# janelia-cosem/fibsem-optflow

Hardware: AMD Instinct MI355X
Metric: slice-pairs/sec (6k×4k, 5 scales, 30 warps) at 1/2/4/8 GPUs; % HBM roofline (higher is better)
Workload: dtype f32; 1 GPU; C2: one 6144x4096 u8 slice pair per GPU per step, nscales 5, warps 30, iterations 300, epsilon 0.01 (reference defaults otherwise); pair=6144x4096, parallelism=pairs sharded over 1 GPU(s), no data-path collective, pairs_in_flight_per_gpu=3, step=one batch of 3 pair(s) solved concurrently per GPU (one ctx + stream each), checks_per_pair=206

## Files before the change

### fibsem-optflow_amd/csrc/tvl1_engine.hip

```cpp
#include <hip/hip_runtime.h>
#include <sched.h>
#include <atomic>
#include <chrono>

#include <cfloat>
#include <cmath>
#include <cstdarg>
#include <cstdio>
#include <cstdlib>
#include <cstring>
#include <string>
#include <vector>

#include "../../include/tvl1.h"
#include "tvl1_plan.hpp"
#include "tvl1_walk.hpp"
#include "tvl1_kernels.hpp"
#include "tvl1_batch.hpp"
#include "tvl1_align_plan.hpp"
#include "tvl1_align.hpp"
#include "tvl1_stack.hpp"
#include "tvl1_shift.hpp"
#include "tvl1_fbcheck.hpp"
#include "tvl1_compose.hpp"
// ... 54 lines not shown
  unsigned long long *gate = nullptr;
  int spec = 1;
  int spec_trace = 0;
  unsigned long long check_seq = 0;
  int poll = 1;
  hipEvent_t ev_order = nullptr;
  hipEvent_t ev_switch = nullptr;
  hipStream_t last_stream = nullptr;
  bool last_stream_valid = false;
  struct Retired {
    char *p;
    std::vector<hipEvent_t> done;
  };
  std::vector<Retired> retired;
  std::vector<hipStream_t> streams;
  int roll_seg = 0;
  long roll_px4_min = 5000000;
  int roll_slots[kRollMax + 1][2][5] = {};
  int fill = 100;
  int fill_shared = 60;
  long roll_long_min = 0;
  int warp_ring_slots = 0;
  size_t buf_limit = ((size_t)1 << 31) - 4096;
  int fuse = 1;
  int tb4 = 1;
  long fuse_min = 4000000;
  int witer_slots = 0;
  int mid = 1;
  double mid_min = 1.1;
  int mid_slots = 0;
  int wi_nc = 2;
  int stages = 1;
  int stage_slots[kRollMax + 1] = {};
  int stages_fill = 0;
  char *barena = nullptr;
  size_t barena_bytes = 0;
  int bW = 0, bH = 0, bL = 0, bn = 0;
  int bws[TVL1_MAX_LEVELS] = {}, bhs[TVL1_MAX_LEVELS] = {};
  float *bI0s[TVL1_MAX_LEVELS] = {}, *bI1s[TVL1_MAX_LEVELS] = {};
  size_t bips[TVL1_MAX_LEVELS] = {};
  float *bU[2][2] = {}, *bP[2][4] = {}, *bC[3] = {};
  size_t bps = 0;
  double *bpartials = nullptr;
  int batch_fuse = 1;
  int batch_group = 1;
  int batch_store_pred = 1;
  int batch_px1_w = kBatchPx1W;
  int kb1_slots[kRollMax + 1] = {};
  int batch_seg_min = 128;
  int probe_lds = 0;
  int probe_wi_lds = 0;
  char *gather_scratch = nullptr;
  size_t gather_bytes = 0;
  int batch_small = 1;
  char *small_scratch = nullptr;
  size_t small_bytes = 0;
  float *map_scratch = nullptr;
  size_t map_bytes = 0;
  char *align_scratch = nullptr;
  size_t align_bytes = 0;
  int4 *align_pat = nullptr;
  char *shift_scratch = nullptr;
  size_t shift_bytes = 0;
  char *seed_scratch = nullptr;
  size_t seed_bytes = 0;
  char *fb_counts = nullptr;
// ... 555 lines not shown
static size_t plane_stride(const tvl1_ctx *c) {
  return (size_t)c->geo.ps[0] * c->geo.H * sizeof(float);
}
static size_t group_bytes(const tvl1_ctx *c, int s, int planes) {
  return (size_t)(planes - 1) * plane_stride(c) + (size_t)c->geo.ps[s] * c->geo.hs[s] * sizeof(float);
}
static bool buffer_ok(const tvl1_ctx *c, int s) {
  return group_bytes(c, s, c->geo.gamma ? 6 : 4) < c->buf_limit;
}
static RollBufs roll_bufs(const tvl1_ctx *c, int s, int uset, int pset, int cbuf) {
  const bool gam = c->geo.gamma;
  RollBufs b;
  b.c = c->C[cbuf][0];
  b.us = c->U[uset][0];
  b.ud = c->U[uset ^ 1][0];
  b.ps = c->Pd[pset][0];
  b.pd = c->Pd[pset ^ 1][0];
  b.pstride = (unsigned)plane_stride(c);
  b.cb = (unsigned)group_bytes(c, s, 3);
  b.ub = (unsigned)group_bytes(c, s, gam ? 3 : 2);
  b.pb = (unsigned)group_bytes(c, s, gam ? 6 : 4);
  return b;
}

struct Level {
  tvl1_ctx *c;
  hipStream_t st;
  int s, lw, lh, P;
  IterArgs a;
  int math;
  bool gam, exact_div;
  bool roll_ok;
  bool roll_long;
};

static tvl1_status gather(const Level &lv, int uset, int cbuf, int wp) {
  tvl1_ctx *c = lv.c;
  hipStream_t st = lv.st;
  const int s = lv.s, lw = lv.lw, lh = lv.lh, P = lv.P;
  size_t t0 = prof_begin(c, st);
  if (!lv.roll_ok) {
    const int tx = (lw + kWarpTW - 1) / kWarpTW, ty = (lh + kWarpTH - 1) / kWarpTH;
#define WARP_IMG(FM)                                                                           \
  hipLaunchKernelGGL(k_warp_img<FM>, dim3(tx * ty), dim3(256), 0, st, c->I0s[s], c->I1s[s],    \
                     c->U[uset][0], c->U[uset][1], lw, lh, P, tx, c->C[cbuf][0], c->C[cbuf][1], \
                     c->C[cbuf][2]);
    MATH_SWITCH(lv.math, WARP_IMG)
#undef WARP_IMG
  } else {
    WarpRingArgs wa;
    wa.I0 = c->I0s[s];
    wa.I1 = c->I1s[s];
    wa.u1 = c->U[uset][0];
    wa.u2 = c->U[uset][1];
    wa.I1wx = c->C[cbuf][0];
    wa.I1wy = c->C[cbuf][1];
    wa.rho = c->C[cbuf][2];
    wa.W = lw;
    wa.H = lh;
    wa.P = P;
    const StreamPlan sp = plan_warp_ring(lw, lh, 6, fill_slots(c->warp_ring_slots, fill_now(c)), c->roll_seg);
    wa.bands = sp.bands;
    wa.seg_rows = sp.seg_rows;
    wa.waves = sp.waves;
#define WARP_RING(FM) \
  hipLaunchKernelGGL((k_warp_ring<6, 2, FM>), dim3(wa.waves), dim3(128), 0, st, wa);
// ... 105 lines not shown
    ROLL_M(kFast, K, PX)                \
  } else if (math == kFma) {            \
    ROLL_M(kFma, K, PX)                 \
  } else {                              \
    ROLL_M(kIEEE, K, PX)                \
  }
#define MID_M(FM) hipLaunchKernelGGL((k_iterate_roll_mid<FM>), grid, dim3(256), 0, st, ra);
  if (midp) {
    MATH_SWITCH(math, MID_M)
  } else if (px == 4) {
    if (k == 1) {
      ROLL(1, 4)
    } else {
      ROLL(2, 4)
    }
  } else {
    switch (k) {
      case 1: ROLL(1, 2) break;
      case 2: ROLL(2, 2) break;
      case 3: ROLL(3, 2) break;
      default: ROLL(4, 2) break;
    }
  }
#undef MID_M
#undef ROLL
#undef ROLL_M
#undef ROLL_G
  *hbm = roll_hbm(sp, lv.lh, k, px, (double)lv.lw * lv.lh, pass_planes(gam, p.p_zero));
  return sp.waves;
}

static bool stages_take(const Level &lv, const PassReq &p) {
  const tvl1_ctx *c = lv.c;
  if (!c->stages || lv.gam || !lv.roll_ok || p.mid || (p.k != 2 && p.k != 4)) return false;
  return c->stages == 2 || (p.k == 4 && !lv.roll_long && c->tb4);
}
static int launch_stages(const Level &lv, const IterArgs &a, const PassReq &p, double *hbm) {
  tvl1_ctx *c = lv.c;
  RollArgs ra;
  ra.b = roll_bufs(c, lv.s, p.ui, p.pi, p.cb);
  ra.it = a;
  const StreamPlan sp =
      plan_stages(lv.lw, lv.lh, p.k,
                  fill_slots(c->stage_slots[p.k], c->stages_fill > 0       ? c->stages_fill
                                                  : fill_now(c) == c->fill ? c->fill
                                                                           : kStagesFillShared),
                  c->roll_seg);
  ra.bands = sp.bands;
  ra.seg_rows = sp.seg_rows;
  ra.waves = sp.waves;
  if (partials_fit(c, sp.waves, sp.waves, "blocks") < 0) return -1;
#define STAGES_M(FM)                                                                        \
  if (p.k == 2)                                                                             \
    hipLaunchKernelGGL((k_iterate_stages<FM, 2>), dim3(sp.waves), dim3(128), 0, lv.st, ra);  \
  else                                                                                      \
    hipLaunchKernelGGL((k_iterate_stages<FM, 4>), dim3(sp.waves), dim3(256), 0, lv.st, ra);
  MATH_SWITCH(lv.math, STAGES_M)
#undef STAGES_M
  *hbm = stages_hbm(sp, lv.lh, p.k, (double)lv.lw * lv.lh, pass_planes(false, p.p_zero));
  return sp.waves;
}

static int launch_tb4(const Level &lv, const IterArgs &a, const PassReq &p, double *hbm) {
  const BlockedPlan bp = tb4_plan(lv.lw, lv.lh, p.k);
  TBArgs t;
  t.it = a;
  t.niter = p.k;
  t.tiles_x = bp.tiles_x;
  t.out_h = bp.out_h;
  const int blocks = bp.blocks;
  if (partials_fit(lv.c, blocks, blocks, "blocks") < 0) return -1;
#define TB4_M(FM) \
  hipLaunchKernelGGL((k_iterate_tb4<FM>), dim3(blocks), dim3(32 * kTb4Groups), 0, lv.st, t);
  MATH_SWITCH(lv.math, TB4_M)
#undef TB4_M
  *hbm = blocked_hbm(blocks, kTb4Groups * kTb4RowsPerThread, (double)lv.lw * lv.lh,
                     pass_planes(lv.gam, p.p_zero));
  return blocks;
}

static int launch_tb(const Level &lv, const IterArgs &a, const PassReq &p, double *hbm) {
  const BlockedPlan bp = tb_plan(lv.lw, lv.lh, p.k);
  TBArgs t;
  t.it = a;
  t.niter = p.k;
  t.tiles_x = bp.tiles_x;
// ... 196 lines not shown
  const bool exact_div = !(taut >= 0.0f && taut <= FLT_MAX);

  int64_t level_iters[TVL1_MAX_LEVELS] = {};
  WalkCounts ct;
  for (int s = L - 1; s >= 0; --s) {
    const int lw = g.ws[s], lh = g.hs[s], P = g.ps[s];
    const double scaledEps = prm.epsilon * prm.epsilon * (double)lw * (double)lh;
    Level lv{};
    lv.c = c;
    lv.st = st;
    lv.s = s;
    lv.lw = lw;
    lv.lh = lh;
    lv.P = P;
    lv.a = iter_args(prm, lw, lh, P, c->partials);
    lv.math = math_of(prm);
    lv.gam = gam;
    lv.exact_div = exact_div;
    lv.roll_ok = buffer_ok(c, s);
    lv.roll_long = lv.roll_ok && (long)((lw + 55) / 56) * ((lh + 31) / 32) >= c->roll_long_min;
    const bool roll_ok = lv.roll_ok;

    WalkLevel wl{};
    wl.level = s;
    wl.warps = prm.warps;
    wl.iterations = prm.iterations;
    wl.kmax = exact_div ? 1 : roll_ok ? kRollMax : kTbMax;
    wl.scaledEps = scaledEps;
    wl.eps_pos = prm.epsilon > 0;
    wl.fuse = c->fuse && !gam && !exact_div && roll_ok && prm.epsilon > 0 && prm.iterations >= 2 &&
              (long)lw * lh >= c->fuse_min;
    wl.median = median;
    wl.spec = c->spec && !exact_div && roll_ok && prm.epsilon > 0;
    wl.mid = c->mid && !gam && !exact_div && lv.roll_long && prm.epsilon > 0 && kRollMax >= 4;
    wl.mid_min = c->mid_min;
    wl.spec_trace = c->spec_trace != 0;
    LevelOps ops{lv, wl, stats};
    ct.level_iters = 0;
    TVL1_TRY(walk_level(ops, wl, ws, ct));
    level_iters[s] = ct.level_iters;
    HIP_TRY(c, hipGetLastError());
    if (s == 0) break;
    TVL1_TRY(upsample(lv, ws.ui));
    ws.ui ^= 1;
  }
  const size_t tk = prof_begin(c, st);
  hipLaunchKernelGGL(k_output, grid2(W, H), kBlk2, 0, st, c->U[ws.ui][0], c->U[ws.ui][1], W, H,
                     g.ps[0], u, v, fpitch);
  prof_end(c, st, tk, 2, (double)W * H * 16.0);
  HIP_TRY(c, hipGetLastError());

  ClassTotals tot;
  if (stats) fill_stats(stats, g, prm.warps, level_iters, ct.checks, ct.spec_misses);
  TVL1_TRY(sum_marks(c, tot));
  if (stats) put_class_totals(stats, tot);
  if (c->spec_trace && ct.mid_passes)
    fprintf(stderr, "mid-check passes %d, ended on the mid state %d\n", ct.mid_passes, ct.mid_taken);
  return TVL1_OK;
}


static tvl1_status ensure_batch(tvl1_ctx *c, int W, int H, int n, hipStream_t st) {
  const Geometry &g = c->geo;
  if (c->barena && c->bW == W && c->bH == H && c->bL == g.L && c->bn >= n &&
      !memcmp(c->bws, g.ws, sizeof(int) * g.L) && !memcmp(c->bhs, g.hs, sizeof(int) * g.L))
    return TVL1_OK;
  const size_t P0 = (size_t)g.ps[0];
  const size_t ps = align_up(P0 * H, 64);
// ... 664 lines not shown
  if (hipGetDeviceCount(&n) != hipSuccess) return 0;
  return n;
}

tvl1_status tvl1_create(tvl1_ctx **out, int device, const tvl1_params *params) {
  if (!out) return set_err(nullptr, TVL1_EINVAL, "out is NULL");
  *out = nullptr;
  tvl1_status s = check_params(nullptr, params);
  if (s != TVL1_OK) return s;
  int n = 0;
  if (hipGetDeviceCount(&n) != hipSuccess || n <= 0)
    return set_err(nullptr, TVL1_ENODEV, "no HIP device visible");
  if (device < 0 || device >= n)
    return set_err(nullptr, TVL1_ENODEV, "device %d out of range (have %d)", device, n);
  hipDeviceProp_t prop;
  if (hipGetDeviceProperties(&prop, device) != hipSuccess)
    return set_err(nullptr, TVL1_ENODEV, "hipGetDeviceProperties failed");
  if (strncmp(prop.gcnArchName, "gfx950", 6) != 0)
    return set_err(nullptr, TVL1_ENODEV, "device %d is %s; this build targets gfx950 only",
                   device, prop.gcnArchName);
  tvl1_ctx *c = new (std::nothrow) tvl1_ctx();
  if (!c) return set_err(nullptr, TVL1_ENOMEM, "out of host memory");
  c->device = device;
  c->prm = *params;
  if (const char *m = getenv("TVL1_ROLL_SEG")) c->roll_seg = atoi(m);
  if (const char *m = getenv("TVL1_ROLL_PX4_MIN")) c->roll_px4_min = atol(m);
  if (const char *m = getenv("TVL1_FUSE")) c->fuse = atoi(m) != 0;
  if (const char *m = getenv("TVL1_MID")) c->mid = atoi(m) != 0;
  if (const char *m = getenv("TVL1_MID_MIN")) c->mid_min = atof(m);
  if (const char *m = getenv("TVL1_WI_NC")) c->wi_nc = atoi(m) == 1 ? 1 : 2;
  if (const char *m = getenv("TVL1_TB4")) c->tb4 = atoi(m) != 0;
  if (const char *m = getenv("TVL1_STAGES")) c->stages = std::min(std::max(atoi(m), 0), 2);
  if (const char *m = getenv("TVL1_STAGES_FILL")) c->stages_fill = std::max(0, atoi(m));
  if (const char *m = getenv("TVL1_POLL")) c->poll = atoi(m);
  if (const char *m = getenv("TVL1_SPEC")) c->spec = atoi(m);
  if (const char *m = getenv("TVL1_SPEC_TRACE")) c->spec_trace = atoi(m);
  if (const char *m = getenv("TVL1_FUSE_MIN")) c->fuse_min = atol(m);
  if (const char *m = getenv("TVL1_BATCH_FUSE")) c->batch_fuse = atoi(m) != 0;
  if (const char *m = getenv("TVL1_BATCH_STORE")) c->batch_store_pred = atoi(m) == 0;
  if (const char *m = getenv("TVL1_BATCH_GROUP")) c->batch_group = atoi(m) != 0;
  if (const char *m = getenv("TVL1_BATCH_PX1_W")) c->batch_px1_w = atoi(m);
  if (const char *m = getenv("TVL1_BATCH_SEG_MIN")) c->batch_seg_min = atoi(m);
  if (const char *m = getenv("TVL1_BATCH_SMALL")) c->batch_small = atoi(m) != 0;
  if (const char *m = getenv("TVL1_PROBE_ROLL_LDS")) c->probe_lds = atoi(m);
  if (const char *m = getenv("TVL1_PROBE_WI_LDS")) c->probe_wi_lds = std::min(atoi(m), 32768);
  if (const char *m = getenv("TVL1_BUF_LIMIT"))
    c->buf_limit = std::min(c->buf_limit, (size_t)std::max(0LL, atoll(m)));
  if (const char *m = getenv("TVL1_CHECK")) c->check = atoi(m);
  if (const char *m = getenv("TVL1_FILL")) c->fill = std::max(10, atoi(m));
  if (const char *m = getenv("TVL1_FILL_SHARED")) c->fill_shared = std::max(10, atoi(m));
  if (hipSetDevice(device) != hipSuccess ||
      hipStreamCreateWithFlags(&c->own_stream, hipStreamNonBlocking) != hipSuccess ||
      hipHostMalloc((void **)&c->pinned, sizeof(double) * (8 + kBatchMax),
                    hipHostMallocMapped | hipHostMallocCoherent) != hipSuccess ||
      hipHostGetDevicePointer((void **)&c->pinned_dev, c->pinned, 0) != hipSuccess ||
      hipEventCreateWithFlags(&c->ev_check[0], hipEventDisableTiming) != hipSuccess ||
      hipEventCreateWithFlags(&c->ev_check[1], hipEventDisableTiming) != hipSuccess ||
      hipMalloc((void **)&c->gate, 256) != hipSuccess ||
      hipMemset(c->gate, 0, 256) != hipSuccess ||
      hipEventCreateWithFlags(&c->ev_order, hipEventDisableTiming) != hipSuccess ||
      hipEventCreateWithFlags(&c->ev_switch, hipEventDisableTiming) != hipSuccess) {
    delete c;
    return set_err(nullptr, TVL1_EHIP, "HIP initialisation failed on device %d", device);
  }
  memset(c->pinned, 0, sizeof(double) * (8 + kBatchMax));
  {
// ... 1287 lines not shown
```

### fibsem-optflow_amd/csrc/tvl1_kernels.hpp

```cpp
#pragma once

#include <hip/hip_runtime.h>
#include <stdint.h>

#include "tvl1_plan.hpp"

#ifdef TVL1_PASSES_TU
#define TVL1_PLAIN template <int TVL1_PASSES_TU_UNUSED = 0>
#else
#define TVL1_PLAIN
#endif

namespace tvl1k {

constexpr int kBlock = 256;
constexpr float kFltEps = 1.1920928955078125e-07f;

__device__ __forceinline__ int imin(int a, int b) { return a < b ? a : b; }
__device__ __forceinline__ int imax(int a, int b) { return a > b ? a : b; }

__device__ __forceinline__ float recip_rn(float d) {
  const float r = __builtin_amdgcn_rcpf(d);
  const float e = __builtin_fmaf(-d, r, 1.0f);
  return __builtin_fmaf(e, r, r);
// ... 2315 lines not shown
                                               float *__restrict__ cring,
                                               float *__restrict__ hring = nullptr) {
  const RollArgs &ra = w.ra;
  const int band = wid % ra.bands, seg = wid / ra.bands;
  const int ys = seg * ra.seg_rows, ye = imin(ys + ra.seg_rows, ra.it.H);
  warp_iter_seg<M, FM, BW, PRIO, NC>(w, band, ys, ye, wid, ring, cring, hring);
}

template <int M, int FM = 0, int BW = 128, int PRIO = 1, int NC = 1>
__global__ __launch_bounds__(64 * NC + BW) void k_warp_iter(WarpIterArgs w) {
  __shared__ float ring[wi_rows<M>() * ring_pitch(wi_ww<M, BW>())];
  __shared__ float cring[2 * 5 * BW];
  __shared__ float hring[NC == 2 ? 2 * kWiH * BW : 1];
  const int wid = __builtin_amdgcn_readfirstlane(xcd_chunk(blockIdx.x, gridDim.x));
  if (wid >= w.ra.waves || gated_off(w.ra.it.gate, w.ra.it.gate_seq)) return;
  warp_iter_body<M, FM, BW, PRIO, NC>(w, wid, ring, cring, hring);
}

constexpr int kStagesH = 6;
constexpr int kStagesBW = 128;
constexpr int kStagesSlot = kStagesH * kStagesBW;
constexpr int kStagesCRow = 3 * kStagesBW;
template <int K>
constexpr int stages_crows() { return K <= 2 ? 4 : 8; }
template <int K>
constexpr int stages_lds_floats() { return stages_crows<K>() * kStagesCRow + (K - 1) * 2 * kStagesSlot; }

struct StageRegs {
  float Uo1[2], Uo2[2];
  float P11p[2], P12p[2], P21p[2], P22p[2];
  float U1p[2], U2p[2];
};

template <int FM, bool LAST>
__device__ __forceinline__ void stage_row(StageRegs &S, const float (&wx)[2], const float (&wy)[2],
                                          const float (&rh)[2], const float (&uo1)[2],
                                          const float (&uo2)[2], const float (&p11)[2],
                                          const float (&p12)[2], const float (&p21)[2],
                                          const float (&p22)[2], float *__restrict__ hout,
                                          const IterArgs &a, const RollBufs &B, int y,
                                          const RollLane &L, unsigned rowb, double &acc) {
  constexpr int PX = 2, BW = kStagesBW;
  const unsigned ps = B.pstride;
  const bool stU = L.out && y >= L.ys && y < L.ye;
  float n1[PX], n2[PX];
#pragma unroll
  for (int j = 0; j < PX; ++j) {
    float n3;
    estimate_u_px<false, FM, false, true>(wx[j], wy[j], rh[j], uo1[j], uo2[j], 0.0f, p11[j],
                                          left_of<PX>(p11, j), p12[j], S.P12p[j], p21[j],
                                          left_of<PX>(p21, j), p22[j], S.P22p[j], 0.0f, 0.0f, 0.0f,
                                          0.0f, L.X + j, y, a, n1[j], n2[j], n3, L.c0);
    if (LAST && a.calc_err) {
      const float e = residual_px<FM>(uo1[j] - n1[j], uo2[j] - n2[j]);
      acc += stU && L.X + j < a.W ? (double)e : 0.0;
    }
  }
  if (LAST) {
    const unsigned vo = stU ? (unsigned)y * rowb + L.vst : kOOB;
    bstorev<PX>(B.ud, B.ub, vo, n1);
    bstorev<PX>(B.ud, B.ub, vo, n2, ps);
  }
  if (y >= a.H) {
#pragma unroll
    for (int j = 0; j < PX; ++j) { n1[j] = S.U1p[j]; n2[j] = S.U2p[j]; }
  }
  const int yD = y - 1;
  float o11[PX], o12[PX], o21[PX], o22[PX];
#pragma unroll
  for (int j = 0; j < PX; ++j) {
    const bool has_right = L.X + j + 1 < a.W;
    dual_px<false, false, FM>(S.U1p[j], right_of<PX>(S.U1p, j), n1[j], has_right, true, a.taut,
                              S.P11p[j], S.P12p[j], o11[j], o12[j], a.taut_small);
    dual_px<false, false, FM>(S.U2p[j], right_of<PX>(S.U2p, j), n2[j], has_right, true, a.taut,
                              S.P21p[j], S.P22p[j], o21[j], o22[j], a.taut_small);
  }
  if (LAST) {
    const unsigned vo = L.out && yD >= L.ys && yD < L.ye ? (unsigned)yD * rowb + L.vst : kOOB;
    bstorev<PX>(B.pd, B.pb, vo, o11);
    bstorev<PX>(B.pd, B.pb, vo, o12, ps);
    bstorev<PX>(B.pd, B.pb, vo, o21, 2 * ps);
    bstorev<PX>(B.pd, B.pb, vo, o22, 3 * ps);
  } else {
    if (yD < 0) {
#pragma unroll
      for (int j = 0; j < PX; ++j) o11[j] = o12[j] = o21[j] = o22[j] = 0.0f;
// ... 3 lines not shown
    lds_put<PX>(hout + 2 * BW, o11);
    lds_put<PX>(hout + 3 * BW, o12);
    lds_put<PX>(hout + 4 * BW, o21);
    lds_put<PX>(hout + 5 * BW, o22);
  }
#pragma unroll
  for (int j = 0; j < PX; ++j) {
    S.U1p[j] = n1[j]; S.U2p[j] = n2[j];
    S.P11p[j] = p11[j]; S.P12p[j] = p12[j]; S.P21p[j] = p21[j]; S.P22p[j] = p22[j];
  }
}

template <int FM, int K>
__device__ __forceinline__ void stage_first_step(StageRegs &S, float *__restrict__ cring,
                                                 float *__restrict__ hring,
                                                 const RollIn<false, 2> &cur, RollIn<false, 2> &ahead,
                                                 const IterArgs &a, const RollBufs &B, int r, int t,
                                                 bool active, const RollLane &L, int lane,
                                                 unsigned rowb) {
  roll_load<false, 2>(ahead, B, (unsigned)imin(r + kRollAhead, a.H - 1) * rowb, L.vload, L.vloadp);
  __builtin_amdgcn_sched_barrier(0);
  lds_barrier();
  if (active) {
    float *c = cring + (r & (stages_crows<K>() - 1)) * kStagesCRow + 2 * lane;
    lds_put<2>(c, cur.wx);
    lds_put<2>(c + kStagesBW, cur.wy);
    lds_put<2>(c + 2 * kStagesBW, cur.rh);
    double none = 0.0;
    stage_row<FM, false>(S, cur.wx, cur.wy, cur.rh, cur.u1, cur.u2, cur.p11, cur.p12, cur.p21,
                         cur.p22, hring + (t & 1) * kStagesSlot + 2 * lane, a, B, r, L, rowb, none);
  }
}

template <int FM, int K, bool LAST>
__device__ __forceinline__ void stage_next_step(StageRegs &S, const float *__restrict__ cring,
                                                const float *__restrict__ hin,
                                                float *__restrict__ hout, const IterArgs &a,
                                                const RollBufs &B, int y, int t, bool active,
                                                const RollLane &L, int lane, unsigned rowb,
                                                double &acc) {
  lds_barrier();
  if (active) {
    constexpr int BW = kStagesBW;
    const float *h = hin + ((t + 1) & 1) * kStagesSlot + 2 * lane;
    float u1[2], u2[2], p11[2], p12[2], p21[2], p22[2], wx[2], wy[2], rh[2];
    lds_get<2>(u1, h);
    lds_get<2>(u2, h + BW);
    lds_get<2>(p11, h + 2 * BW);
    lds_get<2>(p12, h + 3 * BW);
    lds_get<2>(p21, h + 4 * BW);
    lds_get<2>(p22, h + 5 * BW);
    const float *c = cring + (y & (stages_crows<K>() - 1)) * kStagesCRow + 2 * lane;
    lds_get<2>(wx, c);
    lds_get<2>(wy, c + BW);
    lds_get<2>(rh, c + 2 * BW);
    stage_row<FM, LAST>(S, wx, wy, rh, S.Uo1, S.Uo2, p11, p12, p21, p22,
                        LAST ? nullptr : hout + (t & 1) * kStagesSlot + 2 * lane, a, B, y, L, rowb, acc);
#pragma unroll
    for (int j = 0; j < 2; ++j) { S.Uo1[j] = u1[j]; S.Uo2[j] = u2[j]; }
  }
}

template <int FM, int K>
__global__ __launch_bounds__(64 * K) void k_iterate_stages(RollArgs ra) {
  static_assert(K == 2 || K == 4, "one wavefront per iteration of a 2- or 4-iteration pass");
  static_assert(kRollAhead == 2, "the step loops are unrolled for a 3-row ring");
  static_assert(stages_lds_floats<K>() * 4 <= 32768, "5 blocks per CU");
  constexpr int PX = 2, BW = kStagesBW, HALO = roll_halo<K, PX>();
  constexpr int NF = stages_lds_floats<K>();
  __shared__ __attribute__((aligned(16))) float lds[NF];
  const int wid = __builtin_amdgcn_readfirstlane(xcd_chunk(blockIdx.x, gridDim.x));
  if (wid >= ra.waves || gated_off(ra.it.gate, ra.it.gate_seq)) return;
  for (int i = threadIdx.x; i < NF / 4; i += 64 * K)
    reinterpret_cast<float4 *>(lds)[i] = make_float4(0.0f, 0.0f, 0.0f, 0.0f);
  float *cring = lds, *hring = lds + stages_crows<K>() * kStagesCRow;
  const IterArgs &a = ra.it;
  const RollBufs &B = ra.b;
  const int lane = threadIdx.x & 63;
  const int wv = __builtin_amdgcn_readfirstlane(threadIdx.x >> 6);
  const int band = wid % ra.bands, seg = wid / ra.bands;
  const int X0 = band * (BW - 2 * HALO) - HALO;
  RollLane L;
  L.X = X0 + PX * lane;
  L.vload = 4u * imin(imax(L.X, 0), a.P - PX);
  L.vloadp = a.p_zero ? kOOB : L.vload;
  L.out = PX * lane >= HALO && PX * lane < BW - HALO && L.X < a.W;
  L.vst = 4u * (unsigned)imax(L.X, 0);
  L.ys = seg * ra.seg_rows;
  L.ye = imin(L.ys + ra.seg_rows, a.H);
  L.c0 = X0 <= 0;
  const unsigned rowb = 4u * (unsigned)a.P;
  const int r0 = stages_r0(L.ys, K);
  const int thirds = stages_steps(L.ys, L.ye, K) / 3;
  StageRegs S;
#pragma unroll
  for (int j = 0; j < PX; ++j) {
    S.Uo1[j] = S.Uo2[j] = S.U1p[j] = S.U2p[j] = 0.0f;
    S.P11p[j] = S.P12p[j] = S.P21p[j] = S.P22p[j] = 0.0f;
  }
  lds_barrier();
  if (wv == 0) {
    const int yend = L.ye + K - 1;
    RollIn<false, 2> A, Bx, C;
    roll_load<false, 2>(A, B, (unsigned)r0 * rowb, L.vload, L.vloadp);
    roll_load<false, 2>(Bx, B, (unsigned)imin(r0 + 1, a.H - 1) * rowb, L.vload, L.vloadp);
    for (int h = 0, t = 0; h < thirds; ++h, t += 3) {
      progress_prio<1>(h, thirds);
      const int r = r0 + t;
      stage_first_step<FM, K>(S, cring, hring, A, C, a, B, r, t, r <= yend, L, lane, rowb);
      stage_first_step<FM, K>(S, cring, hring, Bx, A, a, B, r + 1, t + 1, r + 1 <= yend, L, lane, rowb);
      stage_first_step<FM, K>(S, cring, hring, C, Bx, a, B, r + 2, t + 2, r + 2 <= yend, L, lane, rowb);
    }
  } else if (wv == K - 1) {
    const float *hin = hring + (K - 2) * 2 * kStagesSlot;
    double acc = 0.0;
    for (int h = 0, t = 0; h < thirds; ++h, t += 3) {
      progress_prio<1>(h, thirds);
#pragma unroll
      for (int i = 0; i < 3; ++i) {
        const int y = r0 + t + i - 2 * (K - 1);
        stage_next_step<FM, K, true>(S, cring, hin, nullptr, a, B, y, t + i, y >= r0 - 1 && y <= L.ye,
                                     L, lane, rowb, acc);
      }
    }
    if (a.calc_err) {
#pragma unroll
      for (int o = 32; o > 0; o >>= 1) acc += __shfl_xor(acc, o);
      if (lane == 0) a.partials[wid] = acc;
    }
  } else if (K > 2) {
    const int n = wv + 1;
    const float *hin = hring + (n - 2) * 2 * kStagesSlot;
    float *hout = hring + (n - 1) * 2 * kStagesSlot;
    const int yend = L.ye + K - n;
    double none = 0.0;
    for (int h = 0, t = 0; h < thirds; ++h, t += 3) {
      progress_prio<1>(h, thirds);
#pragma unroll
      for (int i = 0; i < 3; ++i) {
        const int y = r0 + t + i - 2 * (n - 1);
        stage_next_step<FM, K, false>(S, cring, hin, hout, a, B, y, t + i, y >= r0 - 1 && y <= yend,
                                      L, lane, rowb, none);
      }
    }
  }
}

struct CheckGate {
  const unsigned long long *in;
  unsigned long long in_seq;
  unsigned long long *out;
  double thr;
  int n, iters, kmax, eps_pos;
  int pk, pcalc;
};

TVL1_PLAIN __global__ void k_reduce(const double *__restrict__ partials, int n, double *__restrict__ out,
                         unsigned long long *seq_out, unsigned long long seq, CheckGate g) {
  if (gated_off(g.in, g.in_seq)) return;
  __shared__ double s[kBlock];
  double acc = 0.0;
  for (int i = threadIdx.x; i < n; i += kBlock) acc += partials[i];
  s[threadIdx.x] = acc;
  __syncthreads();
  for (int o = kBlock / 2; o > 0; o >>= 1) {
    if ((int)threadIdx.x < o) s[threadIdx.x] += s[threadIdx.x + o];
    __syncthreads();
  }
  if (threadIdx.x == 0) {
    const double e = s[0];
    out[0] = e;
    if (g.out)
      *g.out = gate_holds(e, g.thr, g.n, g.iters, g.kmax, g.eps_pos, g.pk, g.pcalc) ? seq : 0ull;
    if (seq_out) {
      __threadfence_system();
      *(volatile unsigned long long *)seq_out = seq;
    }
  }
// ... 101 lines not shown
```

### fibsem-optflow_amd/csrc/tvl1_plan.hpp

```cpp
#pragma once

#include <stdint.h>

#include <algorithm>
#include <cfloat>
#include <cmath>
#include <vector>

#include "../../include/tvl1.h"

#if defined(__HIPCC__) || defined(__CUDACC__)
#define TVL1_HD __host__ __device__
#else
#define TVL1_HD
#endif

namespace tvl1k {

constexpr int kWave = 64;
constexpr int kSegPx = (kWave - 2) * 4;
constexpr int kStripRows = 32;
constexpr int kTbMax = 4;
constexpr int kRollMax = 4;
constexpr int kRollMinSeg = 8;
// ... 180 lines not shown
inline double batch_warp_iter_hbm(const StreamPlan &p, int lh, int ww, double Nl, int n, int nz,
                                  int nstore) {
  const double rows = rows_with_halo(lh, p.seg_rows, 2);
  const double band_bytes = (double)p.bands * 128 * rows * 4.0;
  return band_bytes * ((double)nz * 3 + (double)(n - nz) * 7 + (double)n * ww / 128) +
         Nl * 4.0 * (6.0 * n + 3.0 * nstore);
}
inline double roll_hbm(const StreamPlan &p, int lh, int k, int px, double Nl, const PassPlanes &pl) {
  const double rows = rows_with_halo(lh, p.seg_rows, k);
  return (double)p.bands * 64.0 * px * rows * 4.0 * pl.ld + Nl * 4.0 * pl.st;
}
inline double stages_hbm(const StreamPlan &p, int lh, int k, double Nl, const PassPlanes &pl) {
  return roll_hbm(p, lh, k, 2, Nl, pl);
}
inline double batch_roll_hbm(const StreamPlan &p, int lh, int k, int px, double Nl, int n, int nz) {
  const double rows = rows_with_halo(lh, p.seg_rows, k);
  const double band_bytes = (double)p.bands * 64 * px * rows * 4.0;
  return band_bytes * ((double)n * 5 + (double)(n - nz) * 4) + (double)n * Nl * 4.0 * 6.0;
}
inline double blocked_hbm(int blocks, int region_rows, double Nl, const PassPlanes &pl) {
  return (double)blocks * 64.0 * region_rows * 4.0 * pl.ld + Nl * 4.0 * pl.st;
}
inline double iterate_hbm(double Nl, int k, const PassPlanes &pl) { return Nl * 4.0 * (pl.ld + pl.st) * k; }

struct Predictor {
  struct Hist {
    double r0 = -1.0, r1 = -1.0;
    int n0 = -1, n_last = -1;
  };
  int iterations, kmax, warps;
  double scaledEps;
  bool spec_ok, spec_stop_ok, mid;
  double w0_hint;
  std::vector<int> act_prev, act_cur;

  Predictor(int iterations_, int kmax_, double scaledEps_, int warps_, bool spec_ok_,
            bool spec_stop_ok_, bool mid_, double w0_hint_)
      : iterations(iterations_), kmax(kmax_), warps(warps_), scaledEps(scaledEps_), spec_ok(spec_ok_),
        spec_stop_ok(spec_stop_ok_), mid(mid_), w0_hint(w0_hint_),
        act_prev((size_t)std::min(iterations_, 4096) + 1, -2), act_cur(act_prev) {}

  double extrapolate(const Hist &h, int n, int wp) const {
    if (h.r1 < 0) return wp == 0 ? w0_hint : 1.5;
    if (n - h.n_last > 2) return 0.9;
    if (h.r0 >= 0 && h.n_last - h.n0 == 2) return h.r1 * (h.r1 / h.r0);
    return h.n_last == 2 ? h.r1 * 0.6 : h.r1 * 0.93;
  }
  int act_of(double e, int n) const {
    if (!(e > scaledEps && n < iterations)) return 0;
    bool ce;
    double pe;
    return sched_after(e, scaledEps, n, iterations, kmax, 1, &ce, &pe) << 1 | (ce ? 1 : 0);
  }
  void note(Hist &h, double e, int n) {
    h.r0 = h.r1;
    h.n0 = h.n_last;
    h.r1 = e / scaledEps;
    h.n_last = n;
    if ((size_t)n < act_cur.size()) act_cur[n] = act_of(e, n);
  }
  void note_stop_guess(int n) {
    if ((size_t)n < act_cur.size()) act_cur[n] = 0;
  }
  void next_warp() {
    act_prev.swap(act_cur);
    std::fill(act_cur.begin(), act_cur.end(), -2);
  }
  void predict0(int wp, int n, bool alone, bool nostore, int last_n, const Hist &h, bool cur,
                int &pk, int &pcalc) const {
    const std::vector<int> &prevw = cur ? act_cur : act_prev;
    pk = -1;
    pcalc = 0;
    if (!spec_ok) return;
    if (!alone) return;
    const bool can_stop = spec_stop_ok && wp + 1 < warps;
    const bool can_cont = !nostore && n < iterations;
    if (can_stop && (n >= iterations || (n == 2 && last_n == 2))) {
      pk = 0;
      return;
    }
    const int ap = wp >= 2 && n < (int)prevw.size() ? prevw[n] : -2;
    if (ap == 0 && can_stop) {
      pk = 0;
      return;
    }
    if (ap > 0 && can_cont) {
      pk = ap >> 1;
      pcalc = ap & 1;
      return;
    }
    const double r = extrapolate(h, n, wp);
    if (r <= 1.0 && can_stop) {
      pk = 0;
    } else if (can_cont) {
      const int a = act_of(std::max(r, 1.0 + 1e-9) * scaledEps, n);
      pk = a >> 1;
      pcalc = a & 1;
    } else if (can_stop) {
      pk = 0;
    }
  }
  void predict(int wp, int n, bool alone, bool nostore, int last_n, const Hist &h, bool cur, int &pk,
               int &pcalc) const {
    predict0(wp, n, alone, nostore, last_n, h, cur, pk, pcalc);
    if (mid && pk == 2 && pcalc && n > 2) pk = -1;
  }
};

}
```

### fibsem-optflow_amd/csrc/tvl1_walk.hpp

```cpp
#pragma once

#include <cstdio>

#include "tvl1_plan.hpp"

namespace tvl1k {

struct WarpSched {
  int n = 0;
  double error = DBL_MAX, prevError = 0.0;
  struct Next {
    int k;
    bool calc_end;
    double prev_end;
  };
  bool active(double thr, int iterations) const { return error > thr && n < iterations; }
  Next next(double thr, int iterations, int kmax, int eps_pos) const {
    Next p{0, false, prevError};
    p.k = sched_after(prevError, thr, n, iterations, kmax, eps_pos, &p.calc_end, &p.prev_end);
    return p;
  }
  void ran(const Next &p) {
    n += p.k;
    if (p.calc_end) return;
    error = DBL_MAX;
    prevError = p.prev_end;
  }
  void read(double e) { error = prevError = e; }
};

struct PassReq {
  int k;
  bool calc_end;
  int ui, pi, cb;
  bool p_zero, witer, store_c, mid, gated;
  unsigned long long gseq;
};

struct CheckReq {
  int blocks, first;
  bool gated_in;
  unsigned long long in_seq;
  bool gate_out;
  int n, pk, pcalc;
};

struct WalkLevel {
  int level;
  int warps, iterations, kmax;
  double scaledEps;
  int eps_pos;
  bool fuse;
  bool median;
  bool spec;
  bool mid;
  double mid_min;
  bool spec_trace;
};

struct WalkState {
  int ui, pi;
  int cb;
  double w0_hint;
};

struct WalkCounts {
  int64_t checks = 0;
  int32_t spec_misses = 0;
  int mid_passes = 0, mid_taken = 0;
  int64_t level_iters = 0;
};

#define TVL1_WALK_TRY(expr)            \
  do {                                 \
    const tvl1_status r_ = (expr);     \
    if (r_ != TVL1_OK) return r_;      \
  } while (0)

template <class Ops>
class LevelWalk {
 public:
  LevelWalk(Ops &ops, const WalkLevel &lv, WalkState &st, WalkCounts &ct)
      : ops_(ops), lv_(lv), st_(st), ct_(ct),
        pred_(lv.iterations, lv.kmax, lv.scaledEps, lv.warps, lv.spec,
              lv.spec && !lv.median && lv.iterations >= 2, lv.mid, st.w0_hint) {}

  tvl1_status run() {
    for (int wp = 0; wp < lv_.warps; ++wp) TVL1_WALK_TRY(warp(wp));
    return TVL1_OK;
  }

 private:
  using Hist = Predictor::Hist;
  struct Check {
    unsigned long long seq = 0;
    int pk = -1, pcalc = 0;
  };

  Ops &ops_;
  const WalkLevel &lv_;
  WalkState &st_;
  WalkCounts &ct_;
  Predictor pred_;
  bool p_zero_ = true;
  int last_warp_n_ = -1;
  bool pre_ = false, pre_nostore_ = false;
  Check pre_chk_;
  int wp_ = 0;
  WarpSched w_;
  Hist h_;
  bool fused_nostore_ = false;
  bool pending_ = false;
  Check pend_;

  void flip() {
    st_.ui ^= 1;
    st_.pi ^= 1;
    p_zero_ = false;
  }

  tvl1_status warp(int wp) {
    wp_ = wp;
    w_ = WarpSched{};
    h_ = Hist{};
    fused_nostore_ = pending_ = false;
    if (pre_) {
      w_.n = 2;
      fused_nostore_ = pre_nostore_;
      pending_ = true;
      pend_ = pre_chk_;
      pre_ = false;
    } else {
      if (lv_.median) {
        TVL1_WALK_TRY(ops_.median(st_.ui));
        st_.ui ^= 1;
      }
      if (!lv_.fuse) TVL1_WALK_TRY(ops_.gather(st_.ui, st_.cb, wp));
    }
    while (!pre_ && (pending_ || w_.active(lv_.scaledEps, lv_.iterations))) {
      if (!pending_) {
        const WarpSched::Next nx = w_.next(lv_.scaledEps, lv_.iterations, lv_.kmax, lv_.eps_pos);
        if (mid_applies(nx))
          TVL1_WALK_TRY(mid_pass());
        else
          TVL1_WALK_TRY(own_pass(nx));
        if (!pending_) continue;
      }
      TVL1_WALK_TRY(read_check());
    }
    ct_.level_iters += w_.n;
    last_warp_n_ = w_.n;
    ops_.warp_done(wp, w_.n);
    st_.cb ^= 1;
    pred_.next_warp();
    return TVL1_OK;
  }

  tvl1_status own_pass(const WarpSched::Next &nx) {
    const bool witer = lv_.fuse && w_.n == 0 && nx.k == 2 && nx.calc_end;
    const bool store_c = wp_ == 0 || last_warp_n_ != 2;
    int blocks = 0;
    TVL1_WALK_TRY(ops_.pass(PassReq{nx.k, nx.calc_end, st_.ui, st_.pi, st_.cb, p_zero_, witer,
                                    witer && store_c, false, false, 0},
                            wp_, w_.n, &blocks));
    if (witer) fused_nostore_ = !store_c;
    flip();
    w_.ran(nx);
    if (!nx.calc_end) return TVL1_OK;
    pred_.predict(wp_, w_.n, ops_.alone(), fused_nostore_, last_warp_n_, h_, false, pend_.pk, pend_.pcalc);
    TVL1_WALK_TRY(ops_.check(CheckReq{blocks, 0, false, 0, pend_.pk >= 0, w_.n, pend_.pk, pend_.pcalc},
                             &pend_.seq));
    pending_ = true;
    return TVL1_OK;
  }

  bool mid_applies(const WarpSched::Next &nx) const {
    return lv_.mid && nx.k == 2 && nx.calc_end && w_.n > 2 && w_.n + 4 <= lv_.iterations &&
           w_.prevError >= lv_.mid_min * lv_.scaledEps;
  }
  tvl1_status mid_pass() {
    int blocks = 0;
    TVL1_WALK_TRY(ops_.pass(PassReq{4, true, st_.ui, st_.pi, st_.cb, p_zero_, false, false, true, false, 0},
                            wp_, w_.n, &blocks));
    unsigned long long seq_mid = 0, seq_end = 0;
    TVL1_WALK_TRY(ops_.check(CheckReq{blocks, blocks, false, 0, false, 0, -1, 0}, &seq_mid));
    TVL1_WALK_TRY(ops_.check(CheckReq{blocks, 0, false, 0, false, 0, -1, 0}, &seq_end));
    double e = 0.0;
    TVL1_WALK_TRY(ops_.wait(seq_mid, &e));
    w_.n += 2;
    w_.read(e);
    ++ct_.checks;
    pred_.note(h_, e, w_.n);
    ++ct_.mid_passes;
    const WarpSched::Next nx = w_.next(lv_.scaledEps, lv_.iterations, lv_.kmax, 1);
    if (w_.active(lv_.scaledEps, lv_.iterations) && nx.k == 2 && nx.calc_end) {
      TVL1_WALK_TRY(ops_.wait(seq_end, &e));
      w_.n += 2;
      w_.read(e);
      ++ct_.checks;
      pred_.note(h_, e, w_.n);
    } else {
      ++ct_.mid_taken;
      TVL1_WALK_TRY(ops_.pass(PassReq{2, false, st_.ui, st_.pi, st_.cb, false, false, false, false, false, 0},
                              wp_, w_.n - 2, &blocks));
    }
    flip();
    return TVL1_OK;
  }

  tvl1_status speculate(const Check &chk, Check &next, bool &nostore) {
    int blocks = 0;
    if (chk.pk == 0) {
      const int w2 = wp_ + 1, cb2 = st_.cb ^ 1;
      const bool store2 = w_.n != 2;
      if (!lv_.fuse) TVL1_WALK_TRY(ops_.gather(st_.ui, cb2, w2));
      TVL1_WALK_TRY(ops_.pass(PassReq{2, true, st_.ui, st_.pi, cb2, false, lv_.fuse, lv_.fuse && store2,
                                      false, true, chk.seq},
                              w2, 0, &blocks));
      nostore = lv_.fuse && !store2;
      pred_.note_stop_guess(w_.n);
      pred_.predict(w2, 2, ops_.alone(), nostore, w_.n, Hist{}, true, next.pk, next.pcalc);
      TVL1_WALK_TRY(ops_.check(CheckReq{blocks, 0, true, chk.seq, next.pk >= 0, 2, next.pk, next.pcalc},
                               &next.seq));
    } else if (chk.pk > 0) {
      TVL1_WALK_TRY(ops_.pass(PassReq{chk.pk, chk.pcalc != 0, st_.ui, st_.pi, st_.cb, false, false, false,
                                      false, true, chk.seq},
                              wp_, w_.n, &blocks));
      if (chk.pcalc) {
        Hist h2;
        h2.r0 = h_.r1;
        h2.n0 = h_.n_last;
        h2.r1 = h_.r1 < 0 ? -1.0 : pred_.extrapolate(h_, w_.n, wp_);
        h2.n_last = w_.n;
        const int n2 = w_.n + chk.pk;
        pred_.predict(wp_, n2, ops_.alone(), false, last_warp_n_, h2, false, next.pk, next.pcalc);
        TVL1_WALK_TRY(ops_.check(CheckReq{blocks, 0, true, chk.seq, next.pk >= 0, n2, next.pk, next.pcalc},
                                 &next.seq));
      }
    }
    return TVL1_OK;
  }

  tvl1_status read_check() {
    pending_ = false;
    const Check chk = pend_;
    const auto mark = ops_.mark();
    Check next;
    bool nostore = false;
    TVL1_WALK_TRY(speculate(chk, next, nostore));
    double e = 0.0;
    TVL1_WALK_TRY(ops_.wait(chk.seq, &e));
    w_.read(e);
    ++ct_.checks;
    const bool ends = !w_.active(lv_.scaledEps, lv_.iterations);
    if (wp_ == 0 && h_.r1 < 0) st_.w0_hint = pred_.w0_hint = e / lv_.scaledEps;
    pred_.note(h_, e, w_.n);
    const bool right =
        chk.pk >= 0 && gate_holds(e, lv_.scaledEps, w_.n, lv_.iterations, lv_.kmax, 1, chk.pk, chk.pcalc);
    if (lv_.spec_trace) {
      char line[160];
      snprintf(line, sizeof line, "spec level %d warp %d n %d E/thr %.3f guess %d/%d %s\n", lv_.level, wp_,
               w_.n, e / lv_.scaledEps, chk.pk, chk.pcalc, chk.pk < 0 ? "-" : right ? "hit" : "miss");
      ops_.trace(line);
    }
    if (chk.pk >= 0 && !right) {
      ++ct_.spec_misses;
      ops_.rollback(mark);
    }
// ... 31 lines not shown
```

Before: 21.52 slice-pairs/s.

## Run mid-pass convergence checks on the staged k=4 kernel, including each warp's first pass

Adds a k_iterate_stages_mid kernel variant in which a second wavefront also computes the residual after 2 of 4 iterations. This lets the mid-check (one 4-iteration pass that yields errors at both n+2 and n+4) run on the staged path for non-long levels as well as roll-long ones. The walker can now open a warp with a mid pass instead of a fused speculative 2-iteration pass, and the predictor only demotes to mid passes when the extrapolated error is above mid_min. The goal is fewer launches and check round-trips per warp. The cost is extra residual work and partial-buffer space, plus an added gather when a warp starts with a mid pass.

```diff
diff --git a/fibsem-optflow_amd/csrc/tvl1_engine.hip b/fibsem-optflow_amd/csrc/tvl1_engine.hip
--- a/fibsem-optflow_amd/csrc/tvl1_engine.hip
+++ b/fibsem-optflow_amd/csrc/tvl1_engine.hip
@@ -110,6 +110,8 @@
   int wi_nc = 2;
   int stages = 1;
   int stage_slots[kRollMax + 1] = {};
+  int first_mid = 1;
+  long first_mid_min = 4000000;
   int stages_fill = 0;
   char *barena = nullptr;
   size_t barena_bytes = 0;
@@ -731,6 +733,7 @@
   bool gam, exact_div;
   bool roll_ok;
   bool roll_long;
+  bool mid_stages;
 };
 
 static tvl1_status gather(const Level &lv, int uset, int cbuf, int wp) {
@@ -902,8 +905,15 @@
 
 static bool stages_take(const Level &lv, const PassReq &p) {
   const tvl1_ctx *c = lv.c;
-  if (!c->stages || lv.gam || !lv.roll_ok || p.mid || (p.k != 2 && p.k != 4)) return false;
+  if (p.mid) return lv.mid_stages && p.k == 4;
+  if (!c->stages || lv.gam || !lv.roll_ok || (p.k != 2 && p.k != 4)) return false;
   return c->stages == 2 || (p.k == 4 && !lv.roll_long && c->tb4);
+}
+static bool mid_on_stages(const Level &lv) {
+  const tvl1_ctx *c = lv.c;
+  if (!c->first_mid || !c->stages || lv.gam || lv.exact_div || !lv.roll_ok) return false;
+  if (c->first_mid == 2) return c->stages == 2 || (!lv.roll_long && c->tb4);
+  return !lv.roll_long && c->tb4 && (long)lv.lw * lv.lh >= c->first_mid_min;
 }
 static int launch_stages(const Level &lv, const IterArgs &a, const PassReq &p, double *hbm) {
   tvl1_ctx *c = lv.c;
@@ -919,9 +929,15 @@
   ra.bands = sp.bands;
   ra.seg_rows = sp.seg_rows;
   ra.waves = sp.waves;
-  if (partials_fit(c, sp.waves, sp.waves, "blocks") < 0) return -1;
+  if (partials_fit(c, (p.mid ? 2 : 1) * sp.waves, sp.waves, "blocks") < 0) return -1;
+  if (p.mid && (p.k != 4 || !p.calc_end)) {
+    (void)set_err(c, TVL1_EHIP, "internal: mid-check stage pass of k = %d", p.k);
+    return -1;
+  }
 #define STAGES_M(FM)                                                                        \
-  if (p.k == 2)                                                                             \
+  if (p.mid)                                                                                \
+    hipLaunchKernelGGL((k_iterate_stages_mid<FM>), dim3(sp.waves), dim3(256), 0, lv.st, ra); \
+  else if (p.k == 2)                                                                        \
     hipLaunchKernelGGL((k_iterate_stages<FM, 2>), dim3(sp.waves), dim3(128), 0, lv.st, ra);  \
   else                                                                                      \
     hipLaunchKernelGGL((k_iterate_stages<FM, 4>), dim3(sp.waves), dim3(256), 0, lv.st, ra);
@@ -1184,8 +1200,13 @@
               (long)lw * lh >= c->fuse_min;
     wl.median = median;
     wl.spec = c->spec && !exact_div && roll_ok && prm.epsilon > 0;
-    wl.mid = c->mid && !gam && !exact_div && lv.roll_long && prm.epsilon > 0 && kRollMax >= 4;
+    lv.mid_stages = mid_on_stages(lv);
+    wl.mid = c->mid && !gam && !exact_div && (lv.roll_long || lv.mid_stages) && prm.epsilon > 0 &&
+             kRollMax >= 4;
     wl.mid_min = c->mid_min;
+    wl.first_mid = wl.mid && lv.mid_stages && prm.iterations >= 4 && (wl.fuse || c->first_mid == 2);
+    wl.first_mid_force = c->first_mid == 2;
+    wl.mid_gated = lv.mid_stages;
     wl.spec_trace = c->spec_trace != 0;
     LevelOps ops{lv, wl, stats};
     ct.level_iters = 0;
@@ -1916,6 +1937,8 @@
   if (const char *m = getenv("TVL1_TB4")) c->tb4 = atoi(m) != 0;
   if (const char *m = getenv("TVL1_STAGES")) c->stages = std::min(std::max(atoi(m), 0), 2);
   if (const char *m = getenv("TVL1_STAGES_FILL")) c->stages_fill = std::max(0, atoi(m));
+  if (const char *m = getenv("TVL1_FIRST_MID")) c->first_mid = std::min(std::max(atoi(m), 0), 2);
+  if (const char *m = getenv("TVL1_FIRST_MID_MIN")) c->first_mid_min = atol(m);
   if (const char *m = getenv("TVL1_POLL")) c->poll = atoi(m);
   if (const char *m = getenv("TVL1_SPEC")) c->spec = atoi(m);
   if (const char *m = getenv("TVL1_SPEC_TRACE")) c->spec_trace = atoi(m);
diff --git a/fibsem-optflow_amd/csrc/tvl1_kernels.hpp b/fibsem-optflow_amd/csrc/tvl1_kernels.hpp
--- a/fibsem-optflow_amd/csrc/tvl1_kernels.hpp
+++ b/fibsem-optflow_amd/csrc/tvl1_kernels.hpp
@@ -2371,7 +2371,7 @@
   float U1p[2], U2p[2];
 };
 
-template <int FM, bool LAST>
+template <int FM, bool LAST, bool MID = false>
 __device__ __forceinline__ void stage_row(StageRegs &S, const float (&wx)[2], const float (&wy)[2],
                                           const float (&rh)[2], const float (&uo1)[2],
                                           const float (&uo2)[2], const float (&p11)[2],
@@ -2390,7 +2390,7 @@
                                           left_of<PX>(p11, j), p12[j], S.P12p[j], p21[j],
                                           left_of<PX>(p21, j), p22[j], S.P22p[j], 0.0f, 0.0f, 0.0f,
                                           0.0f, L.X + j, y, a, n1[j], n2[j], n3, L.c0);
-    if (LAST && a.calc_err) {
+    if ((LAST && a.calc_err) || MID) {
       const float e = residual_px<FM>(uo1[j] - n1[j], uo2[j] - n2[j]);
       acc += stU && L.X + j < a.W ? (double)e : 0.0;
     }
@@ -2460,7 +2460,7 @@
   }
 }
 
-template <int FM, int K, bool LAST>
+template <int FM, int K, bool LAST, bool MID = false>
 __device__ __forceinline__ void stage_next_step(StageRegs &S, const float *__restrict__ cring,
                                                 const float *__restrict__ hin,
                                                 float *__restrict__ hout, const IterArgs &a,
@@ -2482,21 +2482,21 @@
     lds_get<2>(wx, c);
     lds_get<2>(wy, c + BW);
     lds_get<2>(rh, c + 2 * BW);
-    stage_row<FM, LAST>(S, wx, wy, rh, S.Uo1, S.Uo2, p11, p12, p21, p22,
+    stage_row<FM, LAST, MID>(S, wx, wy, rh, S.Uo1, S.Uo2, p11, p12, p21, p22,
                         LAST ? nullptr : hout + (t & 1) * kStagesSlot + 2 * lane, a, B, y, L, rowb, acc);
 #pragma unroll
     for (int j = 0; j < 2; ++j) { S.Uo1[j] = u1[j]; S.Uo2[j] = u2[j]; }
   }
 }
 
-template <int FM, int K>
-__global__ __launch_bounds__(64 * K) void k_iterate_stages(RollArgs ra) {
+template <int FM, int K, bool MID>
+__device__ __forceinline__ void stages_body(const RollArgs &ra, float *__restrict__ lds) {
   static_assert(K == 2 || K == 4, "one wavefront per iteration of a 2- or 4-iteration pass");
+  static_assert(!MID || K == 4, "the mid check is the one after 2 of 4 iterations");
   static_assert(kRollAhead == 2, "the step loops are unrolled for a 3-row ring");
   static_assert(stages_lds_floats<K>() * 4 <= 32768, "5 blocks per CU");
   constexpr int PX = 2, BW = kStagesBW, HALO = roll_halo<K, PX>();
   constexpr int NF = stages_lds_floats<K>();
-  __shared__ __attribute__((aligned(16))) float lds[NF];
   const int wid = __builtin_amdgcn_readfirstlane(xcd_chunk(blockIdx.x, gridDim.x));
   if (wid >= ra.waves || gated_off(ra.it.gate, ra.it.gate_seq)) return;
   for (int i = threadIdx.x; i < NF / 4; i += 64 * K)
@@ -2556,6 +2556,23 @@
       for (int o = 32; o > 0; o >>= 1) acc += __shfl_xor(acc, o);
       if (lane == 0) a.partials[wid] = acc;
     }
+  } else if (MID && wv == 1) {
+    const float *hin = hring;
+    float *hout = hring + 2 * kStagesSlot;
+    const int yend = L.ye + K - 2;
+    double accm = 0.0;
+    for (int h = 0, t = 0; h < thirds; ++h, t += 3) {
+      progress_prio<1>(h, thirds);
+#pragma unroll
+      for (int i = 0; i < 3; ++i) {
+        const int y = r0 + t + i - 2;
+        stage_next_step<FM, K, false, true>(S, cring, hin, hout, a, B, y, t + i, y >= r0 - 1 && y <= yend,
+                                            L, lane, rowb, accm);
+      }
+    }
+#pragma unroll
+    for (int o = 32; o > 0; o >>= 1) accm += __shfl_xor(accm, o);
+    if (lane == 0) a.partials[ra.waves + wid] = accm;
   } else if (K > 2) {
     const int n = wv + 1;
     const float *hin = hring + (n - 2) * 2 * kStagesSlot;
@@ -2572,6 +2589,18 @@
       }
     }
   }
+}
+
+template <int FM, int K>
+__global__ __launch_bounds__(64 * K) void k_iterate_stages(RollArgs ra) {
+  __shared__ __attribute__((aligned(16))) float lds[stages_lds_floats<K>()];
+  stages_body<FM, K, false>(ra, lds);
+}
+
+template <int FM>
+__global__ __launch_bounds__(256) void k_iterate_stages_mid(RollArgs ra) {
+  __shared__ __attribute__((aligned(16))) float lds[stages_lds_floats<4>()];
+  stages_body<FM, 4, true>(ra, lds);
 }
 
 struct CheckGate {
diff --git a/fibsem-optflow_amd/csrc/tvl1_plan.hpp b/fibsem-optflow_amd/csrc/tvl1_plan.hpp
--- a/fibsem-optflow_amd/csrc/tvl1_plan.hpp
+++ b/fibsem-optflow_amd/csrc/tvl1_plan.hpp
@@ -236,12 +236,16 @@
   double scaledEps;
   bool spec_ok, spec_stop_ok, mid;
   double w0_hint;
+  bool mid_gated;
+  double mid_min;
   std::vector<int> act_prev, act_cur;
 
   Predictor(int iterations_, int kmax_, double scaledEps_, int warps_, bool spec_ok_,
-            bool spec_stop_ok_, bool mid_, double w0_hint_)
+            bool spec_stop_ok_, bool mid_, double w0_hint_, bool mid_gated_ = false,
+            double mid_min_ = 0.0)
       : iterations(iterations_), kmax(kmax_), warps(warps_), scaledEps(scaledEps_), spec_ok(spec_ok_),
-        spec_stop_ok(spec_stop_ok_), mid(mid_), w0_hint(w0_hint_),
+        spec_stop_ok(spec_stop_ok_), mid(mid_), w0_hint(w0_hint_), mid_gated(mid_gated_),
+        mid_min(mid_min_),
         act_prev((size_t)std::min(iterations_, 4096) + 1, -2), act_cur(act_prev) {}
 
   double extrapolate(const Hist &h, int n, int wp) const {
@@ -307,7 +311,9 @@
   void predict(int wp, int n, bool alone, bool nostore, int last_n, const Hist &h, bool cur, int &pk,
                int &pcalc) const {
     predict0(wp, n, alone, nostore, last_n, h, cur, pk, pcalc);
-    if (mid && pk == 2 && pcalc && n > 2) pk = -1;
+    if (mid && pk == 2 && pcalc && n > 2 &&
+        (!mid_gated || (n + 4 <= iterations && extrapolate(h, n, wp) >= mid_min)))
+      pk = -1;
   }
 };
 
diff --git a/fibsem-optflow_amd/csrc/tvl1_walk.hpp b/fibsem-optflow_amd/csrc/tvl1_walk.hpp
--- a/fibsem-optflow_amd/csrc/tvl1_walk.hpp
+++ b/fibsem-optflow_amd/csrc/tvl1_walk.hpp
@@ -56,6 +56,8 @@
   bool mid;
   double mid_min;
   bool spec_trace;
+  bool first_mid, first_mid_force;
+  bool mid_gated;
 };
 
 struct WalkState {
@@ -83,7 +85,8 @@
   LevelWalk(Ops &ops, const WalkLevel &lv, WalkState &st, WalkCounts &ct)
       : ops_(ops), lv_(lv), st_(st), ct_(ct),
         pred_(lv.iterations, lv.kmax, lv.scaledEps, lv.warps, lv.spec,
-              lv.spec && !lv.median && lv.iterations >= 2, lv.mid, st.w0_hint) {}
+              lv.spec && !lv.median && lv.iterations >= 2, lv.mid, st.w0_hint, lv.mid_gated,
+              lv.mid_min) {}
 
   tvl1_status run() {
     for (int wp = 0; wp < lv_.warps; ++wp) TVL1_WALK_TRY(warp(wp));
@@ -124,6 +127,7 @@
     w_ = WarpSched{};
     h_ = Hist{};
     fused_nostore_ = pending_ = false;
+    const bool fm = !pre_ && first_mid_after(wp, last_warp_n_);
     if (pre_) {
       w_.n = 2;
       fused_nostore_ = pre_nostore_;
@@ -135,12 +139,12 @@
         TVL1_WALK_TRY(ops_.median(st_.ui));
         st_.ui ^= 1;
       }
-      if (!lv_.fuse) TVL1_WALK_TRY(ops_.gather(st_.ui, st_.cb, wp));
+      if (!lv_.fuse || fm) TVL1_WALK_TRY(ops_.gather(st_.ui, st_.cb, wp));
     }
     while (!pre_ && (pending_ || w_.active(lv_.scaledEps, lv_.iterations))) {
       if (!pending_) {
         const WarpSched::Next nx = w_.next(lv_.scaledEps, lv_.iterations, lv_.kmax, lv_.eps_pos);
-        if (mid_applies(nx))
+        if (mid_applies(nx) || (fm && w_.n == 0))
           TVL1_WALK_TRY(mid_pass());
         else
           TVL1_WALK_TRY(own_pass(nx));
@@ -154,6 +158,14 @@
     st_.cb ^= 1;
     pred_.next_warp();
     return TVL1_OK;
+  }
+
+  bool first_mid_after(int wp, int prev_n) const {
+    return lv_.first_mid && (lv_.first_mid_force || (wp > 0 && prev_n >= 4));
+  }
+  void guess(int wp, int n, bool nostore, int last_n, const Hist &h, bool cur, Check &c) {
+    pred_.predict(wp, n, ops_.alone(), nostore, last_n, h, cur, c.pk, c.pcalc);
+    if (c.pk == 0 && first_mid_after(wp + 1, n)) c.pk = -1;
   }
 
   tvl1_status own_pass(const WarpSched::Next &nx) {
@@ -167,7 +179,7 @@
     flip();
     w_.ran(nx);
     if (!nx.calc_end) return TVL1_OK;
-    pred_.predict(wp_, w_.n, ops_.alone(), fused_nostore_, last_warp_n_, h_, false, pend_.pk, pend_.pcalc);
+    guess(wp_, w_.n, fused_nostore_, last_warp_n_, h_, false, pend_);
     TVL1_WALK_TRY(ops_.check(CheckReq{blocks, 0, false, 0, pend_.pk >= 0, w_.n, pend_.pk, pend_.pcalc},
                              &pend_.seq));
     pending_ = true;
@@ -179,6 +191,7 @@
            w_.prevError >= lv_.mid_min * lv_.scaledEps;
   }
   tvl1_status mid_pass() {
+    const bool first = w_.n == 0;
     int blocks = 0;
     TVL1_WALK_TRY(ops_.pass(PassReq{4, true, st_.ui, st_.pi, st_.cb, p_zero_, false, false, true, false, 0},
                             wp_, w_.n, &blocks));
@@ -190,10 +203,19 @@
     w_.n += 2;
     w_.read(e);
     ++ct_.checks;
+    if (wp_ == 0 && h_.r1 < 0) st_.w0_hint = pred_.w0_hint = e / lv_.scaledEps;
     pred_.note(h_, e, w_.n);
     ++ct_.mid_passes;
+    if (lv_.spec_trace) {
+      char line[160];
+      snprintf(line, sizeof line, "mid  level %d warp %d n %d E/thr %.3f\n", lv_.level, wp_, w_.n,
+               e / lv_.scaledEps);
+      ops_.trace(line);
+    }
     const WarpSched::Next nx = w_.next(lv_.scaledEps, lv_.iterations, lv_.kmax, 1);
-    if (w_.active(lv_.scaledEps, lv_.iterations) && nx.k == 2 && nx.calc_end) {
+    if (first && w_.active(lv_.scaledEps, lv_.iterations) && !(nx.k == 2 && nx.calc_end)) {
+      w_.ran(w_.next(lv_.scaledEps, lv_.iterations, 2, 1));
+    } else if (w_.active(lv_.scaledEps, lv_.iterations) && nx.k == 2 && nx.calc_end) {
       TVL1_WALK_TRY(ops_.wait(seq_end, &e));
       w_.n += 2;
       w_.read(e);
@@ -201,7 +223,7 @@
       pred_.note(h_, e, w_.n);
     } else {
       ++ct_.mid_taken;
-      TVL1_WALK_TRY(ops_.pass(PassReq{2, false, st_.ui, st_.pi, st_.cb, false, false, false, false, false, 0},
+      TVL1_WALK_TRY(ops_.pass(PassReq{2, false, st_.ui, st_.pi, st_.cb, p_zero_, false, false, false, false, 0},
                               wp_, w_.n - 2, &blocks));
     }
     flip();
@@ -219,7 +241,7 @@
                               w2, 0, &blocks));
       nostore = lv_.fuse && !store2;
       pred_.note_stop_guess(w_.n);
-      pred_.predict(w2, 2, ops_.alone(), nostore, w_.n, Hist{}, true, next.pk, next.pcalc);
+      guess(w2, 2, nostore, w_.n, Hist{}, true, next);
       TVL1_WALK_TRY(ops_.check(CheckReq{blocks, 0, true, chk.seq, next.pk >= 0, 2, next.pk, next.pcalc},
                                &next.seq));
     } else if (chk.pk > 0) {
@@ -233,7 +255,7 @@
         h2.r1 = h_.r1 < 0 ? -1.0 : pred_.extrapolate(h_, w_.n, wp_);
         h2.n_last = w_.n;
         const int n2 = w_.n + chk.pk;
-        pred_.predict(wp_, n2, ops_.alone(), false, last_warp_n_, h2, false, next.pk, next.pcalc);
+        guess(wp_, n2, false, last_warp_n_, h2, false, next);
         TVL1_WALK_TRY(ops_.check(CheckReq{blocks, 0, true, chk.seq, next.pk >= 0, n2, next.pk, next.pcalc},
                                  &next.seq));
       }
```

New measurement: 21.81 slice-pairs/s (median of 6 runs). Within noise of the previous version (+1.4%).
